# AaronWatters/contourist

Hardware: AMD Instinct MI355X
Metric: Mvoxels/s isosurface extraction on 512^3 fp32 grid (higher is better)
Workload: dtype f32

## Files before the change

### contourist_amd/csrc/cx_stream3d.h

```cpp
#pragma once

__device__ __forceinline__ uint32_t cx_task_of_block(const cx_task& T) {
    return (blockIdx.x & 7u) * T.chunk + (blockIdx.x >> 3);
}
struct cx_tile {
    uint32_t k0, j0, p, ib, nrows;
};
__device__ __forceinline__ cx_tile cx_tile_of(const cx_params& P, const cx_task& T, uint32_t b, uint32_t wave) {
    cx_tile t;
    const uint32_t ks = b % T.nks; b /= T.nks;
    const uint32_t jg = b % T.njg;
    const uint32_t ic = b / T.njg;
    t.k0 = ks * 256u;
    t.j0 = jg * (4u * CX_RJ) + wave * CX_RJ;
    t.p = ic * T.ci;
    t.ib = min(t.p + T.ci, P.n0);
    t.nrows = (t.j0 < P.n1) ? min((uint32_t)CX_RJ, P.n1 - t.j0) : 0u;
    return t;
}

#define CX_SQ 512u
#define CX_PLW 260u
#define CX_SBR 32u
static_assert((CX_SWP - 1u) * 1024u / CX_BATCH_MIN + 1u <= CX_SBR, "a streaming wave can close more batches than its LDS stage holds");
static_assert(CX_SQ >= 512u, "half a wave's lanes queue up to 512 cells per step");
template <int DT> struct cx_row4 { typedef float4 v; typedef float h; };
template <> struct cx_row4<CX_DTYPE_U8> { typedef uint32_t v; typedef uint32_t h; };
template <> struct cx_row4<CX_DTYPE_I8> { typedef uint32_t v; typedef uint32_t h; };
template <> struct cx_row4<CX_DTYPE_U16> { typedef cx_v2u v; typedef uint32_t h; };
template <> struct cx_row4<CX_DTYPE_I16> { typedef cx_v2u v; typedef uint32_t h; };
template <> struct cx_row4<CX_DTYPE_F16> { typedef cx_v2u v; typedef uint32_t h; };
template <> struct cx_row4<CX_DTYPE_BF16> { typedef cx_v2u v; typedef uint32_t h; };
template <typename V, size_t AL>
struct __attribute__((packed, aligned(AL))) cx_row4_ua { V v; };
template <int DT>
__device__ __forceinline__ void cx_row4_unpack(const typename cx_row4<DT>::v& w, float& x, float& y, float& z, float& t) {
    if constexpr (sizeof(typename cx_dt<DT>::T) == 1) {
        x = cx_dt<DT>::cvt(w); y = cx_dt<DT>::cvt(w >> 8); z = cx_dt<DT>::cvt(w >> 16); t = cx_dt<DT>::cvt(w >> 24);
    } else {
        x = cx_dt<DT>::cvt(w.x); y = cx_dt<DT>::cvt(w.x >> 16); z = cx_dt<DT>::cvt(w.y); t = cx_dt<DT>::cvt(w.y >> 16);
    }
}
template <bool ALIGNED, int DT>
__device__ __forceinline__ void cx_stream_tile(const cx_params& P, const cx_task& T, const uint32_t b) {
    __shared__ uint32_t s_q[4][CX_SQ];
    __shared__ uint32_t s_br[4][CX_SBR][5];
    extern __shared__ __attribute__((aligned(16))) float s_pl_dyn[];
    __shared__ uint32_t s_tot[4][8];
    __shared__ uint8_t s_ntri[256];
    if (b >= T.nblocks) return;
    s_ntri[threadIdx.x] = cx_d_voxel_ntri[threadIdx.x];
    if (b == 0u && threadIdx.x < 3u && P.torder) P.counters[CX_CNT_TCLS + threadIdx.x] = 0u;
    __syncthreads();
    const uint32_t lane = cx_lane_id();
    const uint32_t wave = __builtin_amdgcn_readfirstlane(threadIdx.x >> 6);
    uint32_t* q = s_q[wave];
    uint32_t ql = 0, qflushed = 0;
    uint32_t nbl = 0, nbflushed = 0;
    const uint32_t w = b * 4u + wave;
    unsigned long long* stamp = P.stamps ? P.stamps + (size_t)w * 4u : nullptr;
    if (stamp && lane == 0) stamp[0] = __builtin_amdgcn_s_memtime();
    const cx_tile tile = cx_tile_of(P, T, b, wave);
    const uint32_t k0 = tile.k0, j0 = tile.j0, ib = tile.ib, nrows = tile.nrows;
    uint32_t p = tile.p;
    uint32_t* __restrict__ gq = P.queue + (size_t)w * T.wcap;
    cx_brec* __restrict__ brec = P.brec + (size_t)w * T.bcap;
    const typename cx_dt<DT>::bits* __restrict__ A = reinterpret_cast<const typename cx_dt<DT>::bits*>(cx_grid_data<DT>(P.grid));
    cx_cnt acc = {0, 0, 0, 0};
    uint32_t qn = 0, qstart = 0, nb = 0;
    uint32_t rv = 0, rt = 0, rc = 0;
    uint32_t nr = 0;
    uint32_t tv = 0;
    bool overflow_t = false;
    float dnear = 3.0e38f;
    cx_fast_geom G;
    G.pstart = p; G.j0 = j0; G.k0 = k0;
    bool overflow = false;
    uint32_t qc = 0;
    const bool interior = (tile.ib < P.n0) && (j0 + (uint32_t)CX_RJ < P.n1) && (k0 + 256u < P.n2);
    auto count_pending = [&]() {
        __builtin_amdgcn_wave_barrier();
        for (uint32_t o0 = qc; o0 < ql; o0 += 64u) {
            const uint32_t o = o0 + lane;
            const bool have = o < ql;
            const uint32_t e = have ? q[o] : 0u;
            uint32_t vm = have ? 0xFFu : 0u;
            if (!interior) {
                uint32_t ci, cj, ck;
                cx_decode_entry(P, G, e, ci, cj, ck);
                vm = have ? cx_corner_valid(P, ci, cj, ck) : 0u;
            }
            const uint32_t sm = cx_entry_signs(e);
            const uint32_t s0 = (sm & 1u) ? 0xFFu : 0u;
            const uint32_t nv = __popc(((sm ^ s0) & vm) & 0xFEu);
            const bool real = (vm == 0xFFu);
            const uint32_t nt = real ? (uint32_t)s_ntri[sm] : 0u;
            acc.v += nv;
            acc.t += nt;
            acc.c += (nv | nt) ? 1u : 0u;
            acc.b += real ? 1u : 0u;
        }
        qc = ql;
    };
    auto flush_queue = [&]() {
        if (!P.tq) count_pending();
        __builtin_amdgcn_wave_barrier();
        if (qflushed + ql <= P.qlimit) {
            for (uint32_t o = lane; o < ql; o += 64u) gq[qflushed + o] = q[o];
            qflushed += ql;
        } else {
            overflow = true;
        }
        __builtin_amdgcn_wave_barrier();
        ql = 0; qc = 0;
    };
    auto flush_brec = [&]() {
        __builtin_amdgcn_wave_barrier();
        if (lane < nbl) {
            cx_brec R;
            R.qoff = s_br[wave][lane][0]; R.n = s_br[wave][lane][1]; R.vpre = s_br[wave][lane][2];
            R.tpre = s_br[wave][lane][3]; R.cpre = s_br[wave][lane][4]; R.near = 0; R.pad0 = 0; R.pad1 = 0;
            brec[nbflushed + lane] = R;
        }
        __builtin_amdgcn_wave_barrier();
        nbflushed += nbl;
        nbl = 0;
    };
    auto close_batch = [&]() {
        if (!P.tq) count_pending();
        const uint32_t bv = cxd_wave_add(acc.v), bt = cxd_wave_add(acc.t), bc = cxd_wave_add(acc.c);
        if (lane == 0) {
            s_br[wave][nbl][0] = qstart; s_br[wave][nbl][1] = qn - qstart; s_br[wave][nbl][2] = rv;
            s_br[wave][nbl][3] = rt; s_br[wave][nbl][4] = rc;
        }
        nbl++; nb++; rv += bv; rt += bt; rc += bc;
        nr += (qn - qstart + 63u) >> 6;
        qstart = qn;
        acc.v = acc.t = acc.c = 0;
    };
    if (nrows != 0u && p < ib) {
        const uint32_t kofs = k0 + 4u * lane;
        const bool lane_valid = kofs < P.n2;
        const uint32_t nvalid = lane_valid ? min(4u, P.n2 - kofs) : 0u;
        const uint32_t kofs_c = (nvalid == 4u) ? kofs : (P.n2 - 4u);
        const uint32_t kshift = kofs - kofs_c;
        const uint32_t last_lane = (uint32_t)__popcll(__ballot(lane_valid)) - 1u;
        const bool halo_in = (k0 + 256u) < P.n2;
        const cx_lmasks LM = cx_lane_masks(P, k0, j0, lane);
        const uint32_t mr = LM.mr, mk = LM.mk, mj = LM.mj;
        (void)mk; (void)mj;

        struct plane_raw {
            typename cx_row4<DT>::v v[CX_RJ + 1];
            typename cx_row4<DT>::h hv[CX_RJ + 1];
        };
        const uint32_t plane_last = min(ib, P.n0 - 1u);
        auto load_plane = [&](uint32_t pp, plane_raw& R) {
            const uint32_t pc = min(pp, plane_last);
#pragma unroll
            for (int r = 0; r <= CX_RJ; r++) {
                const uint32_t jr = min(j0 + (uint32_t)r, P.n1 - 1u);
                const uint32_t rowofs = (pc * P.n1 + jr) * P.n2;
                if constexpr (DT != CX_DTYPE_F32) {
                    typedef typename cx_row4<DT>::v V;
                    R.v[r] = reinterpret_cast<const cx_row4_ua<V, ALIGNED ? sizeof(V) : sizeof(*A)>*>(A + rowofs + kofs_c)->v;
                    R.hv[r] = A[rowofs + (halo_in ? k0 + 256u : 0u)];
                } else {
                R.v[r] = *reinterpret_cast<const float4*>(A + rowofs + kofs_c);
                R.hv[r] = A[rowofs + (halo_in ? k0 + 256u : 0u)];
                }
            }
        };
        float (*ring)[CX_RJ + 1][CX_PLW] = reinterpret_cast<float (*)[CX_RJ + 1][CX_PLW]>(s_pl_dyn + (size_t)wave * (2u * (CX_RJ + 1u) * CX_PLW));
        const bool stage_t = P.tq != nullptr;
        const bool stage_ring = stage_t;
        auto plane_bits = [&](const plane_raw& R, const uint32_t slot) -> uint32_t {
            uint32_t own = 0, halo = 0;
#pragma unroll
            for (int r = CX_RJ; r >= 0; r--) {
                float vx, vy, vz, vw_, hv;
                if constexpr (DT == CX_DTYPE_F32) {
                    vx = R.v[r].x; vy = R.v[r].y; vz = R.v[r].z; vw_ = R.v[r].w; hv = R.hv[r];
                } else {
                    cx_row4_unpack<DT>(R.v[r], vx, vy, vz, vw_);
                    hv = cx_dt<DT>::cvt(R.hv[r]);
                }
                const float vw = vw_;
                if (!ALIGNED) {
                    vx = (kshift == 1u) ? vy : ((kshift == 2u) ? vz : ((kshift == 3u) ? vw : vx));
                    vy = (kshift == 0u) ? vy : ((kshift == 1u) ? vz : vw);
                    vz = (kshift == 0u) ? vz : vw;
                }
                if (stage_ring) {
                    *reinterpret_cast<float4*>(&ring[slot][r][4u * lane]) = make_float4(vx, vy, vz, vw);
                    if (lane == 0u) ring[slot][r][256] = hv;
                }
                const float dx = vx - P.vcmp, dy = vy - P.vcmp, dz = vz - P.vcmp, dw = vw - P.vcmp;
                const float dh = hv - P.vcmp;
                own <<= (CX_ROWBITS - 4u);
                own = __builtin_amdgcn_alignbit(own, __float_as_uint(dw), 31);
                own = __builtin_amdgcn_alignbit(own, __float_as_uint(dz), 31);
                own = __builtin_amdgcn_alignbit(own, __float_as_uint(dy), 31);
                own = __builtin_amdgcn_alignbit(own, __float_as_uint(dx), 31);
                halo <<= (CX_ROWBITS - 1u);
                halo = __builtin_amdgcn_alignbit(halo, __float_as_uint(dh), 31);
                dnear = fminf(dnear, fminf(fminf(fabsf(dx), fabsf(dy)), fminf(fabsf(dz), fminf(fabsf(dw), fabsf(dh)))));
            }
            uint32_t nbr = (uint32_t)__builtin_amdgcn_update_dpp(0, (int)own, 0x130, 0xF, 0xF, false) & CX_M0_MASK;
            if (lane == last_lane) nbr = halo_in ? halo : ((own >> 3) & CX_M0_MASK);
            return own | (nbr << 4);
        };

        plane_raw rawA, rawB;
        load_plane(p, rawB);
        load_plane(p + 1u, rawA);
        uint32_t wprev = plane_bits(rawB, 0u);
        auto step = [&](const plane_raw& cur, plane_raw& nxt) {
            load_plane(p + 2u, nxt);
            const uint32_t wcur = plane_bits(cur, (p + 1u - G.pstart) & 1u);
            const uint32_t op = wprev | (wprev >> 1), ap = wprev & (wprev >> 1);
            const uint32_t oc = wcur | (wcur >> 1), ac = wcur & (wcur >> 1);
            const uint32_t o = op | (op >> CX_ROWBITS) | oc | (oc >> CX_ROWBITS);
            const uint32_t a = ap & (ap >> CX_ROWBITS) & ac & (ac >> CX_ROWBITS);
            const uint32_t act0 = o & ~a & mr;
            if (__ballot(act0 != 0u) != 0ULL) {
                const uint32_t cnt0 = __popc(act0);
                const uint32_t incl0 = cx_wave_incl_scan(cnt0, lane);
                const uint32_t tot = (uint32_t)__builtin_amdgcn_readlane((int)incl0, 63);
                const uint32_t pre = incl0 - cnt0;
                const uint32_t sidx = p - G.pstart;
                const uint32_t ebase = (lane << 15) | (sidx << 21);
                if (P.qa) (P.qa + (size_t)w * (CX_SWP * 64u))[sidx * 64u + lane] =
                    ((qn + pre) << 16) | (act0 & 0xFu) | ((act0 >> 2) & 0xF0u) | ((act0 >> 4) & 0xF00u) | ((act0 >> 6) & 0xF000u);
                const uint32_t nhalf = (tot > CX_SQ) ? 2u : 1u;
                const uint32_t mid = (uint32_t)__builtin_amdgcn_readlane((int)pre, 32);
                const float* __restrict__ plo = &ring[sidx & 1u][0][0];
                const float* __restrict__ phi = &ring[(sidx + 1u) & 1u][0][0];
                float* __restrict__ tqw = stage_t ? P.tq + (size_t)w * T.wcap : nullptr;
                for (uint32_t h = 0; h < nhalf; h++) {
                    const uint32_t cbase = (nhalf == 2u && h == 1u) ? mid : 0u;
                    const uint32_t ctot = (nhalf == 2u) ? (h == 0u ? mid : tot - mid) : tot;
                    if (ql + ctot > CX_SQ) flush_queue();
                    uint32_t act = (nhalf == 1u || (lane >> 5) == h) ? act0 : 0u;
                    uint32_t pos = ql + pre - cbase;
                    while (act) {
                        const uint32_t bit = __ffs(act) - 1u;
                        act &= act - 1u;
                        q[pos++] = ebase | (bit << 10) | ((wprev >> bit) & 0xC3u) | (((wcur >> bit) & 0xC3u) << 2);
                    }
                    __builtin_amdgcn_wave_barrier();
                    for (uint32_t o0 = 0; o0 < (stage_t ? ctot : 0u); o0 += 64u) {
                        const uint32_t o = o0 + lane;
                        const bool have = o < ctot;
                        const uint32_t e = have ? q[ql + o] : 0u;
                        uint32_t ci, cj, ck;
                        cx_decode_entry(P, G, e, ci, cj, ck);
                        const uint32_t vm = have ? cx_corner_valid(P, ci, cj, ck) : 0u;
                        const uint32_t sm = cx_entry_signs(e);
                        const uint32_t s0 = (sm & 1u) ? 0xFFu : 0u;
                        const uint32_t emask = ((sm ^ s0) & vm) & 0xFEu;
                        const uint32_t nv = __popc(emask);
                        const bool real = (vm == 0xFFu);
                        const uint32_t nt = real ? (uint32_t)s_ntri[sm] : 0u;
                        acc.v += nv;
                        acc.t += nt;
                        acc.c += (nv | nt) ? 1u : 0u;
                        acc.b += real ? 1u : 0u;
                        if (stage_t) {
                            const uint32_t bit = (e >> 10) & 31u;
                            const uint32_t rr = (bit * 11u) >> 6;
                            const uint32_t at = rr * CX_PLW + 4u * ((e >> 15) & 63u) + (bit - 6u * rr);
                            float f0 = plo[at], f1 = plo[at + 1u], f2 = plo[at + CX_PLW], f3 = plo[at + CX_PLW + 1u];
                            float f4 = phi[at], f5 = phi[at + 1u], f6 = phi[at + CX_PLW], f7 = phi[at + CX_PLW + 1u];
                            uint32_t vtot;
                            const uint32_t vpre = cx_wave_prefix_small<3>(nv, vtot);
                            if (tv + vtot <= P.tlimit) {
                                asm volatile("" : "+v"(f0), "+v"(f1), "+v"(f2), "+v"(f3), "+v"(f4), "+v"(f5), "+v"(f6), "+v"(f7));
                                const float num = (P.vhi - f0) + P.vlo;
                                const float t1 = cx_fraction(num, f1 - f0), t2 = cx_fraction(num, f2 - f0), t3 = cx_fraction(num, f3 - f0);
                                const float t4 = cx_fraction(num, f4 - f0), t5 = cx_fraction(num, f5 - f0), t6 = cx_fraction(num, f6 - f0);
                                const float t7 = cx_fraction(num, f7 - f0);
                                float* __restrict__ dst = tqw + tv + vpre;
                                if (emask & 0x02u) dst[0] = t1;
                                if (emask & 0x04u) dst[__popc(emask & 0x02u)] = t2;
                                if (emask & 0x08u) dst[__popc(emask & 0x06u)] = t3;
                                if (emask & 0x10u) dst[__popc(emask & 0x0Eu)] = t4;
                                if (emask & 0x20u) dst[__popc(emask & 0x1Eu)] = t5;
                                if (emask & 0x40u) dst[__popc(emask & 0x3Eu)] = t6;
                                if (emask & 0x80u) dst[__popc(emask & 0x7Eu)] = t7;
                            } else {
                                overflow_t = true;
                            }
                            tv += vtot;
                        }
                    }
                    ql += ctot;
                    qn += ctot;
                    __builtin_amdgcn_wave_barrier();
                }
                if (qn - qstart >= CX_BATCH_MIN) close_batch();
            }
            wprev = wcur;
            p++;
        };
        while (p < ib) {
            step(rawA, rawB);
            if (p >= ib) break;
            step(rawB, rawA);
        }
    }
    if (qn > qstart) close_batch();
    flush_queue();
    flush_brec();
    if (stamp && lane == 0) stamp[1] = __builtin_amdgcn_s_memtime();
    cx_run run;
    run.v = rv; run.t = rt; run.c = rc; run.b = cxd_wave_add(acc.b);
    const bool near = __ballot(dnear <= P.near_abs) != 0ULL;
    bool really_near = false;
    if (near && qn != 0u && !overflow) {
        __threadfence();
        cx_run ex = {0, 0, 0, 0, 0};
        cx_process_queue<false, DT>(P, [&](uint32_t x) { return cx_entry_lin(P, G, __builtin_nontemporal_load(gq + x)); }, qn, lane, false, ex, nullptr);
        really_near = !(ex.v == rv && ex.t == rt && ex.c == rc && ex.s == 0u);
        run.b = ex.b;
        if (really_near) { run.v = ex.v; run.t = ex.t; run.c = ex.c; }
    }
    if (overflow_t && qn != 0u && !overflow) really_near = true;
    if (really_near) {
        nb = 1;
        nr = (qn + 63u) >> 6;
        if (lane == 0) {
            cx_brec R;
            R.qoff = 0; R.n = qn; R.vpre = 0; R.tpre = 0; R.cpre = 0; R.near = 1; R.pad0 = 0; R.pad1 = 0;
            brec[0] = R;
        }
    }
    if (lane == 0) {
        cx_wsum S;
        S.nb = nb; S.v = run.v; S.t = run.t; S.c = run.c; S.b = run.b; S.nq = qn; S.near = really_near ? 1u : 0u; S.nr = nr;
        P.wsum[w] = S;
        s_tot[wave][0] = run.v; s_tot[wave][1] = run.t; s_tot[wave][2] = run.c; s_tot[wave][3] = run.b; s_tot[wave][4] = nb;
        s_tot[wave][5] = (really_near && qn != 0u) ? 1u : 0u;
        s_tot[wave][6] = nr;
        s_tot[wave][7] = overflow ? 1u : 0u;
    }
    __syncthreads();
    if (threadIdx.x < 8u) {
        const uint32_t sum = s_tot[0][threadIdx.x] + s_tot[1][threadIdx.x] + s_tot[2][threadIdx.x] + s_tot[3][threadIdx.x];
        uint32_t* cs = P.chunksum + (size_t)(b >> 6) * 8u;
        if (sum) atomicAdd(cs + threadIdx.x, sum);
    }
}
template <bool ALIGNED, int DT>
__global__ __launch_bounds__(256, CX_K1_MIN_WAVES) void cx_k_stream(const cx_params P, const cx_task T) {
    cx_stream_tile<ALIGNED, DT>(P, T, cx_task_of_block(T));
}
#define CX_LEVELS_PER_LAUNCH 8u
struct cx_params_pack {
    cx_params p[CX_LEVELS_PER_LAUNCH];
};
template <bool ALIGNED, int DT>
__global__ __launch_bounds__(256, CX_K1_MIN_WAVES) void cx_k_stream_levels(const cx_params_pack LP, const cx_task T, const uint32_t nlevels) {
    const uint32_t seq = blockIdx.x >> 3;
    const uint32_t tile_seq = seq / nlevels, level = seq - tile_seq * nlevels;
    cx_stream_tile<ALIGNED, DT>(LP.p[level], T, (blockIdx.x & 7u) * T.chunk + tile_seq);
}

__device__ __forceinline__ void cx_scan_list_chunk(const cx_params& P, const cx_task& T, const uint32_t nw, const uint32_t g, const uint32_t nchunks) {
    __shared__ uint32_t s_part[4][8];
    __shared__ uint32_t s_own[4][6];
    const uint32_t tid = threadIdx.x, lane = cx_lane_id(), wave = tid >> 6;
    uint32_t acc[6] = {0, 0, 0, 0, 0, 0}, near_any = 0, rall = 0, over_any = 0;
    for (uint32_t c = tid; c < nchunks; c += 256u) {
        const uint4 lo = *reinterpret_cast<const uint4*>(P.chunksum + (size_t)c * 8u);
        const uint4 hi = *reinterpret_cast<const uint4*>(P.chunksum + (size_t)c * 8u + 4u);
        if (c < g) { acc[0] += lo.x; acc[1] += lo.y; acc[2] += lo.z; acc[3] += lo.w; acc[4] += hi.x; acc[5] += hi.z; }
        near_any |= hi.y;
        rall += hi.z;
        over_any |= hi.w;
    }
    const uint32_t w = g * 256u + tid;
    cx_wsum S;
    S.nb = S.v = S.t = S.c = S.b = S.nq = S.near = S.nr = 0;
    if (w < nw) S = P.wsum[w];
    near_any |= (S.near != 0u && S.nq != 0u) ? 1u : 0u;
    const uint32_t x[6] = {S.v, S.t, S.c, S.b, S.nb, S.nr};
    uint32_t inc[6];
#pragma unroll
    for (int m = 0; m < 6; m++) {
        inc[m] = cx_wave_incl_scan(x[m], lane);
        const uint32_t before = cxd_wave_add(acc[m]);
        if (lane == 63u) { s_own[wave][m] = inc[m]; s_part[wave][m] = before; }
    }
    {
        const uint32_t nr = (__ballot(near_any != 0u) != 0ULL) ? 1u : 0u;
        const uint32_t ra = cxd_wave_add(rall);
        const uint32_t ov = (__ballot(over_any != 0u) != 0ULL) ? 1u : 0u;
        if (lane == 63u) { s_part[wave][6] = nr | (ov << 1); s_part[wave][7] = ra; }
    }
    __syncthreads();
    uint32_t ex[6];
#pragma unroll
    for (int m = 0; m < 6; m++) {
        uint32_t base = s_part[0][m] + s_part[1][m] + s_part[2][m] + s_part[3][m];
        for (uint32_t ww = 0; ww < wave; ww++) base += s_own[ww][m];
        ex[m] = base + inc[m] - x[m];
    }
    const uint32_t rounds = s_part[0][7] + s_part[1][7] + s_part[2][7] + s_part[3][7];
    const uint32_t q = max((rounds + P.nvw - 1u) / P.nvw, CX_S3_MIN_SHARE);
    const uint32_t qk = max((rounds + P.nkw - 1u) / P.nkw, CX_S3_MIN_SHARE);
    if (w < nw) {
        cx_wbase B;
        B.v = ex[0]; B.t = ex[1]; B.c = ex[2]; B.boff = ex[4];
        P.wbase[w] = B;
        const cx_tile tile = cx_tile_of(P, T, w >> 2, w & 3u);
        uint32_t rb = ex[5];
        for (uint32_t i = 0; i < S.nb; i++) {
            if (ex[4] + i >= P.fcap) break;
            const cx_brec R = P.brec[(size_t)w * T.bcap + i];
            cx_bdesc D;
            D.w = w; D.qofs = w * T.wcap + R.qoff; D.n = R.n; D.near = R.near;
            D.vbase = ex[0] + R.vpre; D.tbase = ex[1] + R.tpre; D.cbase = ex[2] + R.cpre; D.rbase = rb;
            D.p = tile.p; D.j0 = tile.j0; D.k0 = tile.k0; D.nsteps = tile.ib - tile.p;
            P.flat[ex[4] + i] = D;
            const uint32_t nrb = (R.n + 63u) >> 6;
            for (uint32_t m = (rb + q - 1u) / q; m * q < rb + nrb; m++) P.rstart[m] = ex[4] + i;
            for (uint32_t m = (rb + qk - 1u) / qk; m * qk < rb + nrb; m++) P.kstart[m] = ex[4] + i;
            rb += nrb;
        }
    }
    if (P.torder) {
        __shared__ uint32_t s_cls[3][4], s_clsbase[3];
        const uint32_t nqp = S.nq + (uint32_t)__shfl_down((int)S.nq, 1);
        const bool isht = !(tid & 1u) && w < nw;
        const uint32_t cls = !isht ? 4u : (nqp >= (P.tile_cap * 5u >> 3) ? 0u : (nqp >= (P.tile_cap * 5u >> 4) ? 1u : (nqp ? 2u : 3u)));
        uint32_t rank = 0;
#pragma unroll
        for (uint32_t c = 0; c < 3u; c++) {
            const uint64_t m = __ballot(cls == c);
            if (cls == c) rank = cx_mbcnt(m);
            if (lane == 0) s_cls[c][wave] = (uint32_t)__popcll(m);
        }
        __syncthreads();
        if (tid < 3u) {
            const uint32_t n = s_cls[tid][0] + s_cls[tid][1] + s_cls[tid][2] + s_cls[tid][3];
            s_clsbase[tid] = n ? atomicAdd(&P.counters[CX_CNT_TCLS + tid], n) : 0u;
        }
        __syncthreads();
        if (cls < 3u) {
            uint32_t at = s_clsbase[cls] + rank;
            for (uint32_t ww = 0; ww < wave; ww++) at += s_cls[cls][ww];
            P.torder[(size_t)cls * (nw >> 1) + at] = w >> 1;
        } else if (cls == 3u) {
            P.bndn[w >> 1] = 0u;
        }
    }
    if (g == nchunks - 1u && tid == 255u) {
        P.counters[CX_CNT_VERTS] = ex[0] + x[0]; P.counters[CX_CNT_TRIS] = ex[1] + x[1];
        P.counters[CX_CNT_CELLS] = ex[2] + x[2]; P.counters[CX_CNT_BORDER] = ex[3] + x[3];
        P.counters[CX_CNT_BATCHES] = ex[4] + x[4];
        P.counters[CX_CNT_ROUNDS] = rounds;
        const uint32_t fl = s_part[0][6] | s_part[1][6] | s_part[2][6] | s_part[3][6];
        P.counters[CX_CNT_NEAR] = fl & 1u;
        P.counters[CX_CNT_OVERFLOW] = (fl >> 1) & 1u;
        P.counters[CX_CNT_TILEOVF] = 0u;
    }
}
__global__ __launch_bounds__(256) void cx_k_scan_list(const cx_params P, const cx_task T, const uint32_t nw) {
    cx_scan_list_chunk(P, T, nw, blockIdx.x, gridDim.x);
}
__global__ __launch_bounds__(256) void cx_k_scan_list_levels(const cx_params* __restrict__ LP, const cx_task T, const uint32_t nw) {
    const cx_params P = LP[blockIdx.y];
    cx_scan_list_chunk(P, T, nw, blockIdx.x, gridDim.x);
}
```

Before: 434,000.

## Load halo per lane once and use uniform scalar row pointers

Previously every lane loaded the same halo value for each of the 5 rows. Now each of the first 5 lanes loads one row's halo, and the per-row halo sign bits are gathered with a ballot and spread with a multiply into the halo mask. Row base pointers are forced wave-uniform through readfirstlane in the global address space, so the per-row address arithmetic runs on scalar registers. The intent is to cut redundant global loads, vector registers and VALU work in the inner plane loop, at the cost of a ballot and hardcoded assumptions on CX_RJ and CX_ROWBITS. The dnear minimum now takes the halo value of the lane's own row instead of all rows, which may change which lanes count as near the surface.

```diff
diff --git a/contourist_amd/csrc/cx_stream3d.h b/contourist_amd/csrc/cx_stream3d.h
--- a/contourist_amd/csrc/cx_stream3d.h
+++ b/contourist_amd/csrc/cx_stream3d.h
@@ -40,6 +40,12 @@
     } else {
         x = cx_dt<DT>::cvt(w.x); y = cx_dt<DT>::cvt(w.x >> 16); z = cx_dt<DT>::cvt(w.y); t = cx_dt<DT>::cvt(w.y >> 16);
     }
+}
+#define CX_GLOBAL __attribute__((address_space(1)))
+__device__ __forceinline__ const CX_GLOBAL char* cx_uniform_ptr(const char* p) {
+    const uint64_t u = reinterpret_cast<uint64_t>(p);
+    const uint32_t lo = __builtin_amdgcn_readfirstlane((uint32_t)u), hi = __builtin_amdgcn_readfirstlane((uint32_t)(u >> 32));
+    return reinterpret_cast<const CX_GLOBAL char*>(((uint64_t)hi << 32) | lo);
 }
 template <bool ALIGNED, int DT>
 __device__ __forceinline__ void cx_stream_tile(const cx_params& P, const cx_task& T, const uint32_t b) {
@@ -152,38 +158,46 @@
 
         struct plane_raw {
             typename cx_row4<DT>::v v[CX_RJ + 1];
-            typename cx_row4<DT>::h hv[CX_RJ + 1];
+            typename cx_row4<DT>::h hv;
         };
         const uint32_t plane_last = min(ib, P.n0 - 1u);
+        constexpr uint32_t esz = (uint32_t)sizeof(*A);
+        const char* const Ab = reinterpret_cast<const char*>(A);
+        uint32_t kbyte = kofs_c * esz;
+        uint32_t hbyte = (min(j0 + min(lane, (uint32_t)CX_RJ), P.n1 - 1u) * P.n2 + min(k0 + 256u, P.n2 - 1u)) * esz;
         auto load_plane = [&](uint32_t pp, plane_raw& R) {
             const uint32_t pc = min(pp, plane_last);
+            asm volatile("" : "+v"(kbyte), "+v"(hbyte));
 #pragma unroll
             for (int r = 0; r <= CX_RJ; r++) {
                 const uint32_t jr = min(j0 + (uint32_t)r, P.n1 - 1u);
                 const uint32_t rowofs = (pc * P.n1 + jr) * P.n2;
+                const CX_GLOBAL char* const rowp = cx_uniform_ptr(Ab + (size_t)rowofs * esz);
                 if constexpr (DT != CX_DTYPE_F32) {
                     typedef typename cx_row4<DT>::v V;
-                    R.v[r] = reinterpret_cast<const cx_row4_ua<V, ALIGNED ? sizeof(V) : sizeof(*A)>*>(A + rowofs + kofs_c)->v;
-                    R.hv[r] = A[rowofs + (halo_in ? k0 + 256u : 0u)];
+                    R.v[r] = reinterpret_cast<const CX_GLOBAL cx_row4_ua<V, ALIGNED ? sizeof(V) : sizeof(*A)>*>(rowp + kbyte)->v;
                 } else {
-                R.v[r] = *reinterpret_cast<const float4*>(A + rowofs + kofs_c);
-                R.hv[r] = A[rowofs + (halo_in ? k0 + 256u : 0u)];
+                const cx_v4f t = *reinterpret_cast<const CX_GLOBAL cx_v4f*>(rowp + kbyte);
+                R.v[r] = make_float4(t.x, t.y, t.z, t.w);
                 }
             }
+            R.hv = *reinterpret_cast<const CX_GLOBAL typename cx_dt<DT>::bits*>(cx_uniform_ptr(Ab + (size_t)(pc * P.n1) * P.n2 * esz) + hbyte);
         };
         float (*ring)[CX_RJ + 1][CX_PLW] = reinterpret_cast<float (*)[CX_RJ + 1][CX_PLW]>(s_pl_dyn + (size_t)wave * (2u * (CX_RJ + 1u) * CX_PLW));
         const bool stage_t = P.tq != nullptr;
         const bool stage_ring = stage_t;
         auto plane_bits = [&](const plane_raw& R, const uint32_t slot) -> uint32_t {
-            uint32_t own = 0, halo = 0;
+            uint32_t own = 0;
+            float hv;
+            if constexpr (DT == CX_DTYPE_F32) hv = R.hv; else hv = cx_dt<DT>::cvt(R.hv);
+            const float dh = hv - P.vcmp;
 #pragma unroll
             for (int r = CX_RJ; r >= 0; r--) {
-                float vx, vy, vz, vw_, hv;
+                float vx, vy, vz, vw_;
                 if constexpr (DT == CX_DTYPE_F32) {
-                    vx = R.v[r].x; vy = R.v[r].y; vz = R.v[r].z; vw_ = R.v[r].w; hv = R.hv[r];
+                    vx = R.v[r].x; vy = R.v[r].y; vz = R.v[r].z; vw_ = R.v[r].w;
                 } else {
                     cx_row4_unpack<DT>(R.v[r], vx, vy, vz, vw_);
-                    hv = cx_dt<DT>::cvt(R.hv[r]);
                 }
                 const float vw = vw_;
                 if (!ALIGNED) {
@@ -193,19 +207,20 @@
                 }
                 if (stage_ring) {
                     *reinterpret_cast<float4*>(&ring[slot][r][4u * lane]) = make_float4(vx, vy, vz, vw);
-                    if (lane == 0u) ring[slot][r][256] = hv;
                 }
                 const float dx = vx - P.vcmp, dy = vy - P.vcmp, dz = vz - P.vcmp, dw = vw - P.vcmp;
-                const float dh = hv - P.vcmp;
                 own <<= (CX_ROWBITS - 4u);
                 own = __builtin_amdgcn_alignbit(own, __float_as_uint(dw), 31);
                 own = __builtin_amdgcn_alignbit(own, __float_as_uint(dz), 31);
                 own = __builtin_amdgcn_alignbit(own, __float_as_uint(dy), 31);
                 own = __builtin_amdgcn_alignbit(own, __float_as_uint(dx), 31);
-                halo <<= (CX_ROWBITS - 1u);
-                halo = __builtin_amdgcn_alignbit(halo, __float_as_uint(dh), 31);
-                dnear = fminf(dnear, fminf(fminf(fabsf(dx), fabsf(dy)), fminf(fabsf(dz), fminf(fabsf(dw), fabsf(dh)))));
+                dnear = fminf(dnear, fminf(fminf(fabsf(dx), fabsf(dy)), fminf(fabsf(dz), fabsf(dw))));
             }
+            static_assert(CX_RJ == 4 && CX_ROWBITS == 6u, "the spread of the halo bits below is written for 5 rows, 6 places apart");
+            const uint32_t hsign = (uint32_t)__ballot((int)__float_as_uint(dh) < 0) & 0x1Fu;
+            const uint32_t halo = (hsign * 0x108421u) & CX_M0_MASK;
+            dnear = fminf(dnear, fabsf(dh));
+            if (stage_ring && lane <= (uint32_t)CX_RJ) ring[slot][lane][256] = hv;
             uint32_t nbr = (uint32_t)__builtin_amdgcn_update_dpp(0, (int)own, 0x130, 0xF, 0xF, false) & CX_M0_MASK;
             if (lane == last_lane) nbr = halo_in ? halo : ((own >> 3) & CX_M0_MASK);
             return own | (nbr << 4);
```

Result: no change. 439,200 (median of 3 runs) (+1.2%).
